# uncommitted6453/kzg-commitments

Hardware: AMD Instinct MI355X
Metric: KZG commits/sec + proofs/sec, BN254 degree-4096 (higher is better)
Workload: dtype u32 (radix-2^29 Montgomery limbs, 254-bit Fp)

## Files before the change

kzg-commitments_amd/csrc/coop.hpp:

```cpp
#pragma once
#include "curve.hpp"

namespace kzgx {

constexpr int COOP_G = 8;
constexpr int COOP_SLOTS = 40;

template <class F>
KZGX_DEV void f29_lds_st(uint32_t* p, const F29<F>& a) {
#pragma unroll
  for (int i = 0; i < F::L; i++) p[i] = a.v[i];
}
template <class F>
KZGX_DEV F29<F> f29_lds_ld(const uint32_t* p) {
  F29<F> a;
#pragma unroll
  for (int i = 0; i < F::L; i++) a.v[i] = p[i];
  return a;
}
KZGX_DEV void coop_fence() { __builtin_amdgcn_fence(__ATOMIC_SEQ_CST, "workgroup"); }

template <class F>
KZGX_DEV F29<F> f29_sel(bool c, const F29<F>& a, const F29<F>& b) {
  F29<F> r;
#pragma unroll
  for (int i = 0; i < F::L; i++) r.v[i] = c ? a.v[i] : b.v[i];
  return r;
}

template <class C>
KZGX_DEV Xyzz<C> coop_dbl(const Xyzz<C>& p, uint32_t* sc, int j) {
  using F = typename C::Fp29;
  constexpr int L = F::L;
  if (xyzz_is_inf<C>(p)) return p;
  uint32_t* b1 = sc;
  uint32_t* b2 = sc + 8 * L;
  uint32_t* b3 = sc + 16 * L;
  const F29<F> U = f29_add<F>(p.Y, p.Y);
  f29_lds_st<F>(b1 + j * L, f29_sqr<F>(f29_sel<F>(j == 0, U, p.X)));
  coop_fence();
  const F29<F> V = f29_lds_ld<F>(b1);
  const F29<F> xx = f29_lds_ld<F>(b1 + L);
  const F29<F> M = f29_add<F>(f29_add<F>(xx, xx), xx);
  {
    const F29<F> A = j == 0 ? U : j == 1 ? p.X : j == 2 ? M : V;
    const F29<F> B = j <= 1 ? V : j == 2 ? M : p.ZZ;
    f29_lds_st<F>(b2 + j * L, f29_mul<F>(A, B));
  }
  coop_fence();
  const F29<F> W = f29_lds_ld<F>(b2);
  const F29<F> S = f29_lds_ld<F>(b2 + L);
  const F29<F> X3 = f29_sub<F>(f29_lds_ld<F>(b2 + 2 * L), f29_add<F>(S, S), F::P4);
  {
    const F29<F> A = f29_sel<F>(j == 0, M, W);
    const F29<F> B = f29_sel<F>(j == 0, f29_sub<F>(S, X3, F::P8), p.ZZZ);
    const F29<F> Cc = f29_sel<F>(j == 0, W, f29_zero<F>());
    const F29<F> D = f29_sel<F>(j == 0, f29_sub<F>(f29_zero<F>(), p.Y, F::P4), f29_zero<F>());
    f29_lds_st<F>(b3 + j * L, f29_mul2<F>(A, B, Cc, D));
  }
  coop_fence();
  Xyzz<C> r;
  r.X = X3;
  r.Y = f29_lds_ld<F>(b3);
  r.ZZ = f29_lds_ld<F>(b2 + 3 * L);
  r.ZZZ = f29_lds_ld<F>(b3 + L);
  coop_fence();
  return r;
}

template <class C>
KZGX_DEV Xyzz<C> coop_add(const Xyzz<C>& p, const Xyzz<C>& q, uint32_t* sc, int j) {
  using F = typename C::Fp29;
  constexpr int L = F::L;
  if (xyzz_is_inf<C>(p)) return q;
  if (xyzz_is_inf<C>(q)) return p;
  uint32_t* b1 = sc;
  uint32_t* b2 = sc + 8 * L;
  uint32_t* b3 = sc + 16 * L;
  uint32_t* b4 = sc + 24 * L;
  uint32_t* bx = sc + 32 * L;
  {
    const F29<F> A = j == 0 ? p.X : j == 1 ? q.X : j == 2 ? p.Y : j == 3 ? q.Y : j == 4 ? p.ZZ : p.ZZZ;
    const F29<F> B = j == 0 ? q.ZZ : j == 1 ? p.ZZ : j == 2 ? q.ZZZ : j == 3 ? p.ZZZ : j == 4 ? q.ZZ : q.ZZZ;
    f29_lds_st<F>(b1 + j * L, f29_mul<F>(A, B));
  }
  coop_fence();
  {
    const int ia = (j & 1) ? 3 : 1;
    const F29<F> x = f29_sub<F>(f29_lds_ld<F>(b1 + ia * L), f29_lds_ld<F>(b1 + (ia - 1) * L), F::P2);
    f29_lds_st<F>(bx + j * L, x);
    f29_lds_st<F>(b2 + j * L, f29_sqr<F>(x));
  }
  coop_fence();
  const F29<F> PP = f29_lds_ld<F>(b2);
  if (f29_is_zero_lt2m<F>(PP)) {
    coop_fence();
    if (f29_is_zero<F>(f29_lds_ld<F>(bx + L))) return coop_dbl<C>(p, sc, j);
    return xyzz_inf<C>();
  }
  {
    const F29<F> A = j == 0 ? f29_lds_ld<F>(bx) : f29_lds_ld<F>(b1 + (j == 1 ? 0 : 4) * L);
    f29_lds_st<F>(b3 + j * L, f29_mul<F>(A, PP));
  }
  coop_fence();
  const F29<F> PPP = f29_lds_ld<F>(b3);
  const F29<F> Q = f29_lds_ld<F>(b3 + L);
  const F29<F> X3 = f29_sub<F>(f29_lds_ld<F>(b2 + L), f29_add<F>(PPP, f29_add<F>(Q, Q)), F::P6);
  {
    const F29<F> A = j == 0 ? f29_lds_ld<F>(bx + L) : f29_lds_ld<F>(b1 + 5 * L);
    const F29<F> B = f29_sel<F>(j == 0, f29_sub<F>(Q, X3, F::P8), PPP);
    const F29<F> Cc = f29_sel<F>(j == 0, f29_sub<F>(f29_zero<F>(), f29_lds_ld<F>(b1 + 2 * L), F::P2), f29_zero<F>());
    const F29<F> D = f29_sel<F>(j == 0, PPP, f29_zero<F>());
    f29_lds_st<F>(b4 + j * L, f29_mul2<F>(A, B, Cc, D));
  }
  coop_fence();
  Xyzz<C> r;
  r.X = X3;
  r.Y = f29_lds_ld<F>(b4);
  r.ZZ = f29_lds_ld<F>(b3 + 2 * L);
  r.ZZZ = f29_lds_ld<F>(b4 + L);
  coop_fence();
  return r;
}

}
```

kzg-commitments_amd/csrc/kzgx_api.hip:

```cpp
#include <hip/hip_runtime.h>

#include <map>
#include <mutex>

#include <array>

#include <algorithm>
#include <cstdlib>
#include <cstring>
#include <new>
#include <random>
#include <string>
#include <vector>

#include "curve_consts.h"
#include "fr_host.hpp"
#include "kzgx_internal.hpp"
#include "kzgx_setup.hpp"

#ifndef KZGX_G2TAB_EAGER_MAX
#define KZGX_G2TAB_EAGER_MAX 16385
#endif

struct kzgx_ctx {
// ... 346 lines not shown
  if (hipGetDeviceCount(&ndev) != hipSuccess || ndev <= 0) return KZGX_ERR_NO_DEVICE;
  if (device < 0 || device >= ndev) return KZGX_ERR_ARG;
  hipDeviceProp_t prop;
  KZGX_TRY_HIP(hipGetDeviceProperties(&prop, device));
  if (std::string(prop.gcnArchName).find("gfx950") == std::string::npos) return KZGX_ERR_NO_DEVICE;
  return KZGX_OK;
}

int setup_finish(kzgx_ctx* ctx);

}

extern "C" {

const char* kzgx_strerror(int s) {
  switch (s) {
    case KZGX_OK: return "ok";
    case KZGX_ERR_ARG: return "invalid argument";
    case KZGX_ERR_HIP: return "HIP runtime error";
    case KZGX_ERR_OOM: return "device out of memory";
    case KZGX_ERR_NO_SRS: return "no SRS loaded";
    case KZGX_ERR_DEGREE: return "polynomial degree be at most one less than the setup size (num_coeffs)";
    case KZGX_ERR_INTERNAL: return "internal error";
    case KZGX_ERR_NO_DEVICE: return "no gfx950 (MI355X) device available";
    case KZGX_ERR_DIV_ZERO: return "division by zero (duplicate interpolation point)";
    default: return "unknown status";
  }
}

int kzgx_base_limbs(int curve) {
  return curve == KZGX_CURVE_BN254 ? 4 : curve == KZGX_CURVE_BLS12381 ? 6 : -1;
}

namespace {
std::mutex g_stream_mu;
std::vector<hipStream_t> g_stream_pool[64];
constexpr size_t STREAM_POOL_MAX = 4;
hipError_t stream_take(int device, hipStream_t* s) {
  if (device >= 0 && device < 64) {
    std::lock_guard<std::mutex> lk(g_stream_mu);
    if (!g_stream_pool[device].empty()) {
      *s = g_stream_pool[device].back();
      g_stream_pool[device].pop_back();
      return hipSuccess;
    }
  }
  return hipStreamCreateWithFlags(s, hipStreamNonBlocking);
}
void stream_give(int device, hipStream_t s) {
  if (!s) return;
  if (device >= 0 && device < 64) {
    std::lock_guard<std::mutex> lk(g_stream_mu);
    if (g_stream_pool[device].size() < STREAM_POOL_MAX) {
      g_stream_pool[device].push_back(s);
      return;
    }
  }
  (void)hipStreamDestroy(s);
}
}

int kzgx_init_device(int curve, int device) {
  if (curve != KZGX_CURVE_BN254 && curve != KZGX_CURVE_BLS12381) return KZGX_ERR_ARG;
  KZGX_TRY(device_ok(device));
  KZGX_TRY_HIP(hipSetDevice(device));
  hipStream_t spare[3] = {nullptr, nullptr, nullptr};
  for (auto& s2 : spare) KZGX_TRY_HIP(stream_take(device, &s2));
  for (auto s2 : spare) stream_give(device, s2);
  hipStream_t st = nullptr;
  KZGX_TRY_HIP(stream_take(device, &st));
  struct StreamGuard {
    hipStream_t s;
    int d;
    ~StreamGuard() {
      (void)hipStreamSynchronize(s);
      stream_give(d, s);
    }
  } sg{st, device};
  int (*const warm[])(hipStream_t) = {
      kzgx::warm_setup,      kzgx::warm_msm,        kzgx::warm_msm_fixed,   kzgx::warm_poly,
      kzgx::warm_srs,        kzgx::warm_pairing,    kzgx::warm_verify_wave, kzgx::warm_latency,
      kzgx::warm_fixed_bn_a, kzgx::warm_fixed_bn_b, kzgx::warm_fixed_bn_c,  kzgx::warm_fixed_bn_d,
      kzgx::warm_fixed_bls_a, kzgx::warm_fixed_bls_b, kzgx::warm_fixed_bls_c, kzgx::warm_fixed_bls_d,
      kzgx::warm_subgroup,   kzgx::warm_msm_joint};
  for (auto f : warm) KZGX_TRY(f(st));
  kzgx::GenTables g;
  KZGX_TRY(kzgx::gen_tables_get(curve, device, st, &g));
  void* h = nullptr;
  KZGX_TRY_HIP(hipHostMalloc(&h, 4096, hipHostMallocMapped | hipHostMallocCoherent));
  (void)hipHostFree(h);
  KZGX_TRY_HIP(hipStreamSynchronize(st));
  return KZGX_OK;
}

int kzgx_create(kzgx_ctx** out, int curve, int device) {
  if (!out || (curve != KZGX_CURVE_BN254 && curve != KZGX_CURVE_BLS12381)) return KZGX_ERR_ARG;
  *out = nullptr;
  KZGX_TRY(device_ok(device));
  kzgx_ctx* ctx = new (std::nothrow) kzgx_ctx();
  if (!ctx) return KZGX_ERR_OOM;
  ctx->c.curve = curve;
  ctx->c.device = device;
  if (const char* e = getenv("KZGX_WINDOW_BITS")) {
    int c = atoi(e);
    if (kzgx::window_bits_supported(c)) ctx->c.c = c;
  }
  ctx->c.W = (257 + ctx->c.c - 1) / ctx->c.c;
  ctx->c.fixed.joint.g_req = -1;
  if (const char* e = getenv("KZGX_FIXED_JOINT")) {
    const int g = atoi(e);
    if (g == -1 || g == 0 || (g >= 2 && g <= 25)) ctx->c.fixed.joint.g_req = g;
  }
  if (const char* e = getenv("KZGX_FIXED_JOINT_RANGES")) {
    const int r = atoi(e);
    if (r >= 0 && r <= 8) ctx->c.fixed.joint.ranges = (uint32_t)r;
  }
  hipError_t e = hipSetDevice(device);
  if (e == hipSuccess) e = stream_take(device, &ctx->c.stream);
  if (e != hipSuccess) {
    delete ctx;
    return kzgx::hip_fail(e);
  }
  kzgx::ctx_live_add(device, +1);
  *out = ctx;
  return KZGX_OK;
}

int kzgx_release_cached_memory(int device) {
  if (device < 0 || device >= 64) return KZGX_ERR_ARG;
  int prev = 0;
  KZGX_TRY_HIP(hipGetDevice(&prev));
  KZGX_TRY_HIP(hipSetDevice(device));
  kzgx::table_cache_release();
  return hipSetDevice(prev) == hipSuccess ? KZGX_OK : KZGX_ERR_HIP;
}

int kzgx_shared_tables(int device, size_t* count, size_t* bytes) {
  if (!count || !bytes || device < 0 || device >= 64) return KZGX_ERR_ARG;
  kzgx::shared_tables_info(device, count, bytes);
  return KZGX_OK;
}

void kzgx_destroy(kzgx_ctx* ctx) {
  if (!ctx) return;
  (void)hipSetDevice(ctx->c.device);
  (void)hipStreamSynchronize(ctx->c.stream);
  (void)kzgx_prof_clear(ctx);
  Ctx& c = ctx->c;
  void* bufs[] = {c.d_table, c.d_table_small, c.d_table_big, c.d_inf, c.d_stage[0], c.d_stage[1], c.d_stage[2], c.d_stage[3],
                  c.d_poly_ws, c.d_poly_ws2, ctx->d_srs_canon, ctx->d_srs2_canon, c.d_g2_ws, ctx->d_vw, ctx->d_g2tab,
                  c.d_lift, c.d_ntt_tw};
  for (void* p : bufs)
    if (p) (void)hipFree(p);
  for (void* p : ctx->d_chk)
    if (p) (void)hipFree(p);
  for (auto& f : c.fk) {
    if (f.x) (void)hipFree(f.x);
    if (f.inf) (void)hipFree(f.inf);
    if (f.ev) (void)hipEventDestroy(f.ev);
  }
  for (auto& row : c.fkm)
    for (auto& f : row) {
      if (f.x) (void)hipFree(f.x);
      if (f.inf) (void)hipFree(f.inf);
      if (f.ev) (void)hipEventDestroy(f.ev);
    }
  kzgx::fixed_free(&c);
// ... 2087 lines not shown
```

kzg-commitments_amd/csrc/kzgx_internal.hpp:

```cpp
#pragma once
#include <hip/hip_runtime.h>
#include <stddef.h>
#include <stdint.h>

#include <cstdlib>
#include <vector>

#include "../../include/kzg_gpu.h"

#ifndef KZGX_ACCUM_WAVES
#define KZGX_ACCUM_WAVES 3
#endif

#ifndef KZGX_BS_WAVES
#define KZGX_BS_WAVES 2
#endif

#ifndef KZGX_WINDOW_BITS
#define KZGX_WINDOW_BITS 12
#endif

#define KZGX_TRY(expr)                 \
  do {                                 \
    int _rc = (expr);                  \
// ... 185 lines not shown
      if (w.bound_at < lru->bound_at) lru = &w;
    if (lru->done_recorded && hipEventSynchronize(lru->done) != hipSuccess) return WsLease(this, nullptr, st);
    lru->done_recorded = false;
    lru->owner = st;
    lru->bound_at = ++ws_clock;
    return WsLease(this, lru, st);
  }
  void ws_release(MsmWs* w, hipStream_t st) {
    if (!w->done && hipEventCreateWithFlags(&w->done, hipEventDisableTiming) != hipSuccess) {
      w->done = nullptr;
      (void)hipStreamSynchronize(st);
      return;
    }
    w->done_recorded = hipEventRecord(w->done, st) == hipSuccess;
    if (!w->done_recorded) (void)hipStreamSynchronize(st);
  }
  bool prof_on = false;
  std::vector<ProfRec> prof;
  void* d_poly_ws = nullptr;
  size_t poly_ws_b = 0;
  void* d_poly_ws2 = nullptr;
  size_t poly_ws2_b = 0;
  void* d_g2_ws = nullptr;
  size_t g2_ws_b = 0;
  uint32_t* d_lift = nullptr;
  size_t lift_b = 0;
  uint32_t* d_ntt_tw = nullptr;
  size_t ntt_tw_b = 0;
  int ntt_log2 = -1;
  hipEvent_t ntt_ev = nullptr;
  FkSetup fk[NTT_MAX_LOG2];
  FkSetup fkm[NTT_MAX_LOG2 + 1][NTT_MAX_LOG2 + 1];
  void* d_stage[4] = {nullptr, nullptr, nullptr, nullptr};
  size_t stage_b[4] = {0, 0, 0, 0};
  int base_words() const { return curve == KZGX_CURVE_BN254 ? 8 : 12; }
};

inline WsLease::~WsLease() {
  if (w_) c_->ws_release(w_, st_);
}

struct ProfScope {
  Ctx* ctx;
  hipStream_t st;
  ProfRec rec;
  ProfScope(Ctx* c, hipStream_t s, const char* name) : ctx(c), st(s) {
    rec.name = nullptr;
    if (!ctx->prof_on) return;
    rec.name = name;
    (void)hipEventCreate(&rec.a);
    (void)hipEventCreate(&rec.b);
    (void)hipEventRecord(rec.a, st);
  }
  ~ProfScope() {
    if (!rec.name) return;
    (void)hipEventRecord(rec.b, st);
    ctx->prof.push_back(rec);
  }
};

int dev_alloc(Ctx* ctx, void** p, size_t bytes, size_t* cap);

bool window_bits_supported(int c);
bool fixed_bits_supported(int c);
int fixed_windows(int curve, int c);
int fixed_build(Ctx* ctx, const uint32_t* d_canon, size_t n_srs);
int fixed_build_table(Ctx* ctx, FixedTable& ft, const uint32_t* d_canon, size_t n_srs);
int fixed_rebuild_default(Ctx* ctx, const uint32_t* d_canon, size_t n_srs);
void fixed_free(Ctx* ctx);
void fixed_free_table(FixedTable& ft);
bool fixed_usable(const Ctx* ctx, size_t n);
bool fixed_table_usable(const FixedTable& ft, size_t n);
int fixed_msm_table(Ctx* ctx, FixedTable& ft, const uint32_t* d_scalars, size_t n, size_t batch, size_t stride_words,
                    uint32_t* d_out, uint32_t* d_out_inf, hipStream_t st, uint32_t* xyzz_out);
int fixed_msm(Ctx* ctx, const uint32_t* d_scalars, size_t n, size_t batch, size_t stride_words, uint32_t* d_out,
              uint32_t* d_out_inf, hipStream_t st, uint32_t* xyzz_out);
size_t joint_table_bytes(int curve, int g, size_t n);
int joint_plan(int curve, int c, size_t n, int g_req, int* g, int* c_win);
int joint_build(Ctx* ctx, JointTable& jt, const uint32_t* d_canon, size_t n, int g);
void joint_free(JointTable& jt);
bool joint_serves(const FixedTable& ft, size_t n, size_t batch, bool xyzz_out);
int joint_msm(Ctx* ctx, FixedTable& ft, const uint32_t* d_scalars, size_t n, size_t batch, size_t stride_words,
              uint32_t* d_out, uint32_t* d_out_inf, hipStream_t st);
int srs_upload(Ctx* ctx, const uint32_t* d_canon, size_t n);
int microbench_mixed_add(Ctx* ctx, double* rate);
int microbench_mad_u64(Ctx* ctx, double* rate, double* ghz);
int clock_probe(Ctx* ctx, hipStream_t st, uint32_t spin_us, uint64_t* d_out);
size_t fixed_table_bytes(int curve, int c, size_t n);
int debug_latency(Ctx* ctx, int op, uint32_t iters, double* res);
int xyzz_sum(Ctx* ctx, const uint32_t* d_parts, size_t count, uint32_t* d_out, uint32_t* d_out_inf, hipStream_t st);
int msm_batch(Ctx* ctx, const uint32_t* d_scalars, size_t n, size_t batch, size_t stride_words, uint32_t* d_out,
              uint32_t* d_out_inf, hipStream_t st);
struct PointSeg {
  const uint32_t* xy;
  const uint32_t* inf;
  size_t n;
};
constexpr size_t MSM_POINTS_MAX = KZGX_MSM_POINTS_MAX;
int msm_points(Ctx* ctx, MsmWs& ws, const PointSeg* segs, int nseg, const uint32_t* d_scalars, uint32_t* d_out,
               uint32_t* d_out_inf, hipStream_t st);
int aggregate_scalars(Ctx* ctx, const uint32_t* d_z, const uint32_t* d_y, const uint32_t* d_r, size_t n,
                      uint32_t* d_out, hipStream_t st);
size_t cells_fold_slices(size_t count, unsigned log2l);
int cells_scalars(Ctx* ctx, const uint32_t* d_T, const uint32_t* d_r, const uint32_t* d_cell_index,
                  const uint32_t* d_commit_index, size_t count, size_t n_commits, unsigned log2l, unsigned log2D,
                  bool bitrev, uint32_t* d_out, uint32_t* d_gate, hipStream_t st);
int msm_partial_xyzz(Ctx* ctx, const uint32_t* d_scalars, size_t n, uint32_t* d_rec, hipStream_t st);
int gen_srs_points(Ctx* ctx, const uint32_t* tau_canon_host, size_t start, size_t n, uint32_t* d_out_canon,
                   hipStream_t st);
int g1_validate(Ctx* ctx, const uint32_t* d_xy, uint32_t* d_ok, hipStream_t st);
int g1_sum(Ctx* ctx, const uint32_t* d_xy, const uint32_t* d_inf, size_t count, uint32_t* d_out, uint32_t* d_out_inf,
           hipStream_t st);

int quotient_single(Ctx* ctx, const uint32_t* d_coeffs, size_t n, size_t coeff_stride_words, const uint32_t* d_z,
                    size_t batch, uint32_t* d_q, size_t q_stride_words, uint32_t* d_y, hipStream_t st);
int poly_eval(Ctx* ctx, const uint32_t* d_coeffs, size_t n, const uint32_t* d_x, size_t m, uint32_t* d_y,
              hipStream_t st);
int poly_vanishing(Ctx* ctx, const uint32_t* d_x, size_t n, uint32_t* d_Z, hipStream_t st);
int prove_range_poly(Ctx* ctx, const uint32_t* d_P, size_t n, const uint32_t* d_x, size_t len, uint32_t* d_q,
                     size_t* nq, hipStream_t st);
int poly_interpolate(Ctx* ctx, const uint32_t* d_x, const uint32_t* d_y, size_t n, uint32_t* d_coeffs,
                     hipStream_t st);
int verify_ws_reserve(Ctx* ctx, size_t n);
int g2_ws_reserve(Ctx* ctx, size_t n);

int ntt_max_log2(int curve);
int ntt(Ctx* ctx, const uint32_t* d_in, size_t in_stride, uint32_t* d_out, size_t out_stride, unsigned log2n,
        size_t batch, bool inverse, bool bitrev, hipStream_t st);
int ntt_twiddles(Ctx* ctx, unsigned log2n, hipStream_t st);

int g1_ntt(Ctx* ctx, MsmWs& ws, const uint32_t* d_in_xy, const uint32_t* d_in_inf, uint32_t* d_out_xy,
           uint32_t* d_out_inf, unsigned log2n, size_t batch, bool inverse, bool bitrev, hipStream_t st);
int prove_all_setup(Ctx* ctx, MsmWs& ws, const uint32_t* d_srs_canon, unsigned log2n, hipStream_t st);
int prove_all(Ctx* ctx, MsmWs& ws, const uint32_t* d_srs_canon, const uint32_t* d_coeffs, size_t stride,
              unsigned log2n, size_t batch, bool bitrev, uint32_t* d_out_xy, uint32_t* d_out_inf, hipStream_t st);
void prove_all_drop(Ctx* ctx);
int prove_cosets_setup(Ctx* ctx, MsmWs& ws, const uint32_t* d_srs_canon, unsigned log2n, unsigned log2l,
                       hipStream_t st);
int prove_cosets(Ctx* ctx, MsmWs& ws, const uint32_t* d_srs_canon, const uint32_t* d_coeffs, size_t stride,
                 unsigned log2n, unsigned log2l, size_t batch, bool ext, bool bitrev, uint32_t* d_out_xy,
                 uint32_t* d_out_inf, uint32_t* d_y, hipStream_t st);

constexpr size_t RECOVER_CHUNK_SCALARS = KZGX_RECOVER_CHUNK_SCALARS;
int recover_cells(Ctx* ctx, MsmWs& ws, const uint32_t* d_blob_index, const uint32_t* d_cell_index,
                  const uint32_t* d_ys, size_t count, size_t n_blobs, size_t b0, size_t cb, unsigned log2n,
                  unsigned log2l, bool bitrev, bool want_coef, uint32_t* d_out_y, uint32_t* d_out_coeffs,
                  uint32_t* d_ok, hipStream_t st);

int gen_srs_g2_points(Ctx* ctx, const uint32_t* d_tau, size_t start, size_t n, uint32_t* d_out, hipStream_t st);
size_t g2_table_bytes(int curve, size_t n);
int g2_table_build(Ctx* ctx, const uint32_t* d_srs2, size_t n, uint32_t* d_tab, hipStream_t st);
int msm_g2(Ctx* ctx, const uint32_t* d_scalars, const uint32_t* d_srs2, size_t n, uint32_t* d_out,
           uint32_t* d_out_inf, hipStream_t st,
           const uint32_t* d_tab = nullptr);
int g2_validate(Ctx* ctx, const uint32_t* d_xy, size_t count, uint32_t* d_ok, hipStream_t st);
int pairing_batch(Ctx* ctx, const uint32_t* d_g1, const uint32_t* d_g1_inf, const uint32_t* d_g2,
                  const uint32_t* d_g2_inf, size_t count, uint32_t* d_out, hipStream_t st);
int verify_single_batch(Ctx* ctx, const uint32_t* d_commits, const uint32_t* d_commit_inf, const uint32_t* d_proofs,
                        const uint32_t* d_proof_inf, const uint32_t* d_z, const uint32_t* d_y, size_t count,
                        const uint32_t* d_g1_0, const uint32_t* d_g2_01, uint32_t* d_ok, hipStream_t st);
size_t verify_wave_bytes(int curve);
int verify_wave_prepare(Ctx* ctx, const uint32_t* d_g1_0, const uint32_t* d_g2_01, const uint32_t* g1_comb,
                        uint32_t* d_buf, hipStream_t st);
int verify_wave_batch(Ctx* ctx, const uint32_t* d_commits, const uint32_t* d_commit_inf, const uint32_t* d_proofs,
                      const uint32_t* d_proof_inf, const uint32_t* d_z, const uint32_t* d_y, size_t count,
                      const uint32_t* d_g1_0, const uint32_t* d_buf, uint32_t* d_ok, hipStream_t st);
// ... 18 lines not shown
```

kzg-commitments_amd/csrc/kzgx_setup.hpp:

```cpp
#pragma once
#include <hip/hip_runtime.h>

#include <cstddef>
#include <cstdint>

namespace kzgx {

int warm_setup(hipStream_t st);
int warm_msm(hipStream_t st);
int warm_msm_fixed(hipStream_t st);
int warm_poly(hipStream_t st);
int warm_srs(hipStream_t st);
int warm_pairing(hipStream_t st);
int warm_verify_wave(hipStream_t st);
int warm_latency(hipStream_t st);
int warm_subgroup(hipStream_t st);
int warm_msm_joint(hipStream_t st);
int warm_fixed_bn_a(hipStream_t st);
int warm_fixed_bn_b(hipStream_t st);
int warm_fixed_bn_c(hipStream_t st);
int warm_fixed_bn_d(hipStream_t st);
int warm_fixed_bls_a(hipStream_t st);
int warm_fixed_bls_b(hipStream_t st);
int warm_fixed_bls_c(hipStream_t st);
int warm_fixed_bls_d(hipStream_t st);

struct GenTables {
  uint32_t* g1_comb = nullptr;
  uint32_t* g2_comb = nullptr;
};
constexpr int GEN_COMB_ENTRIES = 32 * 255;
int gen_tables_get(int curve, int device, hipStream_t st, GenTables* out);

int gen_srs_g1_comb(int curve, const uint32_t* d_tau, size_t start, size_t n, const uint32_t* g1_comb,
                    uint32_t* d_out, hipStream_t st);
int gen_srs_g2_comb(int curve, const uint32_t* d_tau, size_t start, size_t n, const uint32_t* g2_comb,
                    uint32_t* d_out, hipStream_t st);

int fixed_multiples_batch(int curve, const uint32_t* d_bases, const uint8_t* d_inf, uint32_t n, int W, uint32_t H,
                          size_t is, size_t ws, uint32_t* d_tab, hipStream_t st);

int vtab_prepare(int curve, const uint32_t* d_g1_0, const uint32_t* g1_comb, uint32_t* d_vtab, hipStream_t st);

int g1_fold_packed(int curve, const uint32_t* d_rec, size_t count, uint32_t* d_out, hipStream_t st);
#ifndef KZGX_G2_TAB_BITS
#define KZGX_G2_TAB_BITS 8
#endif
constexpr int G2_TAB_BITS = KZGX_G2_TAB_BITS;
static_assert(G2_TAB_BITS == 4 || G2_TAB_BITS == 8 || G2_TAB_BITS == 16, "digits must tile a 32-bit word");
constexpr int G2_TAB_WINDOWS = 256 / G2_TAB_BITS;
int g2_table_comb(int curve, const uint32_t* d_tau, size_t start, size_t n, const uint32_t* g2_comb, uint32_t* d_tab,
                  hipStream_t st);
size_t xyzz_record_words(int curve);
int g1_fold_xyzz(int curve, const uint32_t* d_rec, size_t count, uint32_t* d_out, hipStream_t st);
int affine_to_xyzz(int curve, const uint32_t* d_xy, const uint32_t* d_inf, uint32_t* d_rec, hipStream_t st);

int vw_bench(int curve, int op, uint32_t iters, double* ns_per_op, double* clk_per_op, hipStream_t st);

size_t big_reduce_rt_bytes(int curve, uint32_t nb);
int big_reduce(int curve, const uint32_t* d_offsets, uint32_t nb, const uint32_t* d_bsum, uint32_t* d_rt,
               uint32_t* d_out, uint32_t* d_out_inf, hipStream_t st, uint32_t* xyzz_out = nullptr);
int big_reduce_seg(int curve, const uint32_t* d_seg_off, uint32_t* d_part, uint32_t nb, uint32_t s_ub,
                   const uint32_t* d_flag, uint32_t* d_rt, uint32_t* d_out, uint32_t* d_out_inf, hipStream_t st,
                   uint32_t* xyzz_out = nullptr);

}
```

kzg-commitments_amd/csrc/msm_joint.hip:

```cpp
#include <hip/hip_runtime.h>

#include <algorithm>

#include "curve.hpp"
#include "fixed_accum.hpp"
#include "fixed_msm.hpp"
#include "kzgx_internal.hpp"
#include "kzgx_setup.hpp"

namespace kzgx {

constexpr uint32_t JOINT_PL = 256;
constexpr uint32_t JOINT_NEG = 1u << 31;

__host__ __device__ static inline int joint_split(int m) { return m < 4 ? m : (m / 2 > 4 ? m / 2 : 4); }

template <class F>
KZGX_DEV void f29_store_words(uint32_t* p, const F29<F>& a) {
#pragma unroll
  for (int i = 0; i < F::L; i++) p[i] = a.v[i];
}
template <class F>
KZGX_DEV F29<F> f29_load_words(const uint32_t* p) {
  F29<F> r;
#pragma unroll
  for (int i = 0; i < F::L; i++) r.v[i] = p[i];
  return r;
}

size_t joint_table_bytes(int curve, int g, size_t n) {
  if (g < 2 || n == 0) return 0;
  const size_t pb = curve == KZGX_CURVE_BN254 ? packed_words<BN254G1>() * 4 : packed_words<BLS12381G1>() * 4;
  return (n + g - 1) / g * ((size_t)1 << (g - 1)) * pb;
}

template <class C>
__global__ __launch_bounds__(64) void k_joint_halves(const uint32_t* __restrict__ canon, uint32_t n_t, uint32_t g,
                                                     uint32_t blocks, uint32_t la_max, uint32_t hs,
                                                     uint32_t* __restrict__ half) {
  constexpr int AW = affine_words<C>();
  const uint64_t t = (uint64_t)blockIdx.x * blockDim.x + threadIdx.x;
  if (t >= (uint64_t)blocks * hs) return;
  const uint32_t b = (uint32_t)(t / hs), e = (uint32_t)(t % hs);
  const uint32_t p0 = b * g;
  const uint32_t gb = n_t - p0 < g ? n_t - p0 : g;
  const int m = (int)gb - 1, a = joint_split(m);
  const bool hi = e >= la_max;
  const uint32_t j = hi ? e - la_max : e;
  const int cnt = hi ? m - a : a;
  if (j >= (1u << cnt)) return;
  Xyzz<C> acc = xyzz_inf<C>();
  Affine<C> p;
  if (hi && affine_from_canonical<C>(canon + (size_t)(p0 + m) * 2 * C::Fp::N, p)) acc = xyzz_from_affine<C>(p);
  const uint32_t first = p0 + (hi ? (uint32_t)a : 0u);
  for (int i = 0; i < cnt; i++) {
    if (!affine_from_canonical<C>(canon + (size_t)(first + i) * 2 * C::Fp::N, p)) continue;
    if (!((j >> i) & 1u)) p = affine_neg<C>(p);
    acc = xyzz_add_affine<C>(acc, p);
  }
  xyzz_to_affine<C>(acc, p);
  affine_store<C>(half + ((size_t)b * hs + e) * AW, p);
}

template <class C>
KZGX_DEV bool affine_is_inf(const Affine<C>& a) {
  using F = typename C::Fp29;
  return f29_is_zero_exact<F>(a.x) && f29_is_zero_exact<F>(a.y);
}

template <class C>
KZGX_PT bool joint_entry_exact(const Affine<C>& hb, const Affine<C>& la, Affine<C>& out) {
  Xyzz<C> s = affine_is_inf<C>(hb) ? xyzz_inf<C>() : xyzz_from_affine<C>(hb);
  if (!affine_is_inf<C>(la)) s = xyzz_add_affine<C>(s, la);
  return xyzz_to_affine<C>(s, out);
}

template <class C>
__global__ __launch_bounds__(64) void k_joint_entries_small(const uint32_t* __restrict__ half, uint32_t b0,
                                                            uint32_t nb, int m, uint32_t la_max, uint32_t hs,
                                                            size_t bstride, uint32_t* __restrict__ tab,
                                                            unsigned long long* __restrict__ n_inf) {
  constexpr int AW = affine_words<C>();
  constexpr int PW = packed_words<C>();
  const int a = joint_split(m);
  const uint64_t t = (uint64_t)blockIdx.x * blockDim.x + threadIdx.x;
  if (t >= ((uint64_t)nb << m)) return;
  const uint32_t b = b0 + (uint32_t)(t >> m), j = (uint32_t)(t & ((1u << m) - 1u));
  const uint32_t* H = half + (size_t)b * hs * AW;
  Affine<C> r;
  const bool fin = joint_entry_exact<C>(affine_load<C>(H + (size_t)(la_max + (j >> a)) * AW),
                                        affine_load<C>(H + (size_t)(j & ((1u << a) - 1u)) * AW), r);
  if (!fin) atomicAdd(n_inf, 1ull);
  packed_store<C>(tab + (size_t)b * bstride + (size_t)j * PW, r);
}

// ... 178 lines not shown
  constexpr int BITS = C::SCALAR_BITS;
  const uint32_t b = blockIdx.y, lane = threadIdx.x;
  const uint32_t hi = lane >> 5, li = lane & 31u;
  const uint32_t blk = 2 * blockIdx.x + hi;
  uint32_t gb = 0;
  if (blk < nb) gb = n_t - blk * g < g ? n_t - blk * g : g;
  const uint32_t i = blk * g + li;
  uint32_t s[8] = {0, 0, 0, 0, 0, 0, 0, 0};
  if (li < gb && i < n) scalar_load(scalars + (size_t)b * stride_words + (size_t)i * 8, s);
  scalar_reduce<C>(s);
  const uint32_t flip = odd_prepare<C>(s);
  s[(BITS - 1) >> 5] |= 1u << ((BITS - 1) & 31);
  const uint32_t keep = li < gb ? ~0u : 0u;
#pragma unroll
  for (int k = 0; k < 8; k++) s[k] = (s[k] ^ (0u - flip)) & keep;
  const uint32_t low = gb ? (1u << (gb - 1)) - 1u : 0u;
  uint32_t* out = idx + ((size_t)b * nb + blk) * JOINT_PL + li;
#pragma unroll
  for (int k = 0; k < 8; k++) {
    uint32_t mine = s[k];
    auto swap = [&](int j, uint32_t m) __attribute__((always_inline)) {
      const uint32_t p = __shfl_xor(mine, j, 64);
      mine = (li & (uint32_t)j) ? (((p >> j) & m) | (mine & ~m)) : ((mine & m) | ((p & m) << j));
    };
    swap(16, 0x0000ffffu);
    swap(8, 0x00ff00ffu);
    swap(4, 0x0f0f0f0fu);
    swap(2, 0x33333333u);
    swap(1, 0x55555555u);
    if (gb) {
      const uint32_t top = (mine >> (gb - 1)) & 1u;
      out[32 * k] = ((top ? mine : ~mine) & low) | (top ? 0u : JOINT_NEG);
    }
  }
}

template <class C, bool INF, int V = madd_variant<C>()>
__global__ __launch_bounds__(64, fixed_accum_waves<C>()) void k_joint_accum(
    const uint32_t* __restrict__ idx, uint32_t nb, uint32_t per, const uint32_t* __restrict__ tab, size_t bstride,
    uint32_t R, uint32_t* __restrict__ part) {
  constexpr int XW = xyzz_words<C>();
  constexpr int PW = packed_words<C>();
  const uint32_t b = blockIdx.y, rho = blockIdx.x >> 2;
  const uint32_t w = (blockIdx.x & 3u) * 64 + threadIdx.x;
  if (w >= (uint32_t)C::SCALAR_BITS) return;
  const uint32_t b0 = rho * per, b1 = b0 + per < nb ? b0 + per : nb;
  Xyzz<C> acc = xyzz_inf<C>();
  if (b0 < b1) {
    const uint32_t last = b1 - 1;
    const uint32_t* ip = idx + (size_t)b * nb * JOINT_PL + w;
    auto fetch = [&](uint32_t blk, uint32_t word) __attribute__((always_inline)) {
      return packed_fetch<C>(tab + (size_t)blk * bstride + (size_t)(word & ~JOINT_NEG) * PW);
    };
    uint32_t wq = ip[(size_t)b0 * JOINT_PL];
    PackedPt<C> pq = fetch(b0, wq);
    uint32_t wn = ip[(size_t)(b0 + 1 < last ? b0 + 1 : last) * JOINT_PL];
#pragma unroll 1
    for (uint32_t blk = b0; blk < b1; blk++) {
      Affine<C> cur = packed_unpack<C>(pq);
      const uint32_t neg = wq >> 31;
      const uint32_t nx = blk + 1 < last ? blk + 1 : last;
      wq = wn;
      pq = fetch(nx, wq);
      wn = ip[(size_t)(blk + 2 < last ? blk + 2 : last) * JOINT_PL];
      const bool skip = INF && affine_is_inf<C>(cur);
      affine_cond_neg<C>(cur, neg);
      const Xyzz<C> sum = xyzz_add_affine_v<C, V>(acc, cur);
      if constexpr (INF) {
#pragma unroll
        for (int k = 0; k < C::Fp29::L; k++) {
          acc.X.v[k] = skip ? acc.X.v[k] : sum.X.v[k];
          acc.Y.v[k] = skip ? acc.Y.v[k] : sum.Y.v[k];
          acc.ZZ.v[k] = skip ? acc.ZZ.v[k] : sum.ZZ.v[k];
          acc.ZZZ.v[k] = skip ? acc.ZZZ.v[k] : sum.ZZZ.v[k];
        }
      } else {
        acc = sum;
      }
    }
  }
  xyzz_store<C>(part + (((size_t)b * R + rho) * JOINT_PL + w) * XW, acc);
}

template <class C>
__global__ __launch_bounds__(64) void k_joint_horner1(const uint32_t* __restrict__ part, uint32_t count,
                                                      uint32_t* __restrict__ segs) {
  constexpr int XW = xyzz_words<C>();
  constexpr uint32_t BITS = C::SCALAR_BITS;
  const uint32_t t = blockIdx.x * blockDim.x + threadIdx.x;
  if (t >= count * 8) return;
  const uint32_t br = t >> 3, seg = t & 7u;
  const uint32_t lo = 32 * seg, hi = lo + 32 < BITS ? lo + 32 : BITS;
  const uint32_t* p = part + (size_t)br * JOINT_PL * XW;
  Xyzz<C> acc = xyzz_load<C>(p + (size_t)(hi - 1) * XW);
  for (uint32_t w = hi - 1; w-- > lo;) {
    const Xyzz<C> a = xyzz_load<C>(p + (size_t)w * XW);
    acc = xyzz_dbl<C>(acc);
    acc = xyzz_add<C>(acc, a);
  }
  xyzz_store<C>(segs + (size_t)t * XW, acc);
}

template <class C>
__global__ __launch_bounds__(64) void k_joint_horner2(const uint32_t* __restrict__ segs, uint32_t batch, uint32_t R,
                                                      uint32_t* __restrict__ sums) {
  constexpr int XW = xyzz_words<C>();
  const uint32_t b = blockIdx.x * blockDim.x + threadIdx.x;
  if (b >= batch) return;
  const uint32_t* p = segs + (size_t)b * R * 8 * XW;
  Xyzz<C> acc = xyzz_inf<C>();
  for (int seg = 7; seg >= 0; seg--) {
    if (seg < 7)
      for (int k = 0; k < 32; k++) acc = xyzz_dbl<C>(acc);
    for (uint32_t r = 0; r < R; r++) acc = xyzz_add<C>(acc, xyzz_load<C>(p + ((size_t)r * 8 + seg) * XW));
  }
  xyzz_store<C>(sums + (size_t)b * XW, acc);
}

bool joint_serves(const FixedTable& ft, size_t n, size_t batch, bool xyzz_out) {
  const JointTable& jt = ft.joint;
  if (!jt.d || xyzz_out || n == 0 || n > jt.n_t) return false;
  return jt.g_req >= 2 ? batch >= 1 : batch >= 64;
}

template <class C>
static int joint_msm_impl(Ctx* ctx, FixedTable& ft, const uint32_t* d_scalars, size_t n, size_t batch,
                          size_t stride_words, uint32_t* d_out, uint32_t* d_out_inf, hipStream_t st) {
  const JointTable& jt = ft.joint;
  constexpr size_t XB = xyzz_words<C>() * sizeof(uint32_t);
  static_assert(C::SCALAR_BITS <= (int)JOINT_PL && C::SCALAR_BITS > 224, "4 wavefronts and 8 segments of planes");
  const uint32_t nb = (uint32_t)((n + jt.g - 1) / jt.g);
  uint32_t R = jt.ranges ? jt.ranges : 1u;
  R = std::min(R, nb);
  const uint32_t per = (nb + R - 1) / R;
  if (batch > 65535 || 4 * (size_t)R > 65535) return KZGX_ERR_ARG;
  WsLease wsp = ctx->ws_for(st);
  if (!wsp) return KZGX_ERR_ARG;
  MsmWs& ws = *wsp;
  KZGX_TRY(dev_alloc(ctx, (void**)&ws.jidx, batch * (size_t)nb * JOINT_PL * 4, &ws.jidx_b));
  KZGX_TRY(dev_alloc(ctx, (void**)&ws.fpart, batch * (size_t)R * JOINT_PL * XB, &ws.fpart_b));
  KZGX_TRY(dev_alloc(ctx, (void**)&ws.fsum, batch * ((size_t)R * 8 + 1) * XB, &ws.fsum_b));
  {
    ProfScope p(ctx, st, "msm_scatter");
    hipLaunchKernelGGL(k_joint_index<C>, dim3((nb + 1) / 2, (unsigned)batch), dim3(64), 0, st, d_scalars, (uint32_t)n,
                       stride_words, (uint32_t)jt.n_t, (uint32_t)jt.g, nb, ws.jidx);
  }
  {
    ProfScope p(ctx, st, "msm_accum");
    const size_t bstride = ((size_t)1 << (jt.g - 1)) * packed_words<C>();
    if (jt.n_inf)
      hipLaunchKernelGGL((k_joint_accum<C, true>), dim3(4 * R, (unsigned)batch), dim3(64), 0, st, ws.jidx, nb, per,
                         jt.d, bstride, R, ws.fpart);
    else
      hipLaunchKernelGGL((k_joint_accum<C, false>), dim3(4 * R, (unsigned)batch), dim3(64), 0, st, ws.jidx, nb, per,
                         jt.d, bstride, R, ws.fpart);
  }
  {
    ProfScope p(ctx, st, "msm_reduce");
    uint32_t* sums = ws.fsum + batch * (size_t)R * 8 * xyzz_words<C>();
    hipLaunchKernelGGL(k_joint_horner1<C>, dim3((unsigned)((batch * R * 8 + 63) / 64)), dim3(64), 0, st, ws.fpart,
                       (uint32_t)(batch * R), ws.fsum);
    hipLaunchKernelGGL(k_joint_horner2<C>, dim3((unsigned)((batch + 63) / 64)), dim3(64), 0, st, ws.fsum,
                       (uint32_t)batch, R, sums);
    fixed_finish_launch<C>(sums, (uint32_t)batch, d_out, d_out_inf, nullptr, st);
  }
  KZGX_TRY_HIP(hipGetLastError());
  return KZGX_OK;
}

int joint_msm(Ctx* ctx, FixedTable& ft, const uint32_t* d_scalars, size_t n, size_t batch, size_t stride_words,
              uint32_t* d_out, uint32_t* d_out_inf, hipStream_t st) {
  return ctx->curve == KZGX_CURVE_BN254
             ? joint_msm_impl<BN254G1>(ctx, ft, d_scalars, n, batch, stride_words, d_out, d_out_inf, st)
             : joint_msm_impl<BLS12381G1>(ctx, ft, d_scalars, n, batch, stride_words, d_out, d_out_inf, st);
}

__global__ void k_warm_msm_joint() {}
int warm_msm_joint(hipStream_t st) {
  hipLaunchKernelGGL(k_warm_msm_joint, dim3(1), dim3(64), 0, st);
  KZGX_TRY_HIP(hipGetLastError());
  return KZGX_OK;
}

}
```

Before: 284,800.

## Split joint Horner into 16 segments and cooperative 8-lane final reduce

The joint MSM's Horner reduction now splits the 256 bit-planes into 16 segments of 16 instead of 8 of 32, doubling parallelism in the first pass. The second pass, previously one thread per batch item running serial doublings and adds, now uses groups of 8 lanes that cooperate on each point doubling and addition through LDS. This shortens the serial tail that leaves the GPU underused at small batch. The cost is more segment partials to combine, LDS fences on every group operation, and a separate compile unit that needs special memory-clause flags.

```diff
diff --git a/kzg-commitments_amd/csrc/coop.hpp b/kzg-commitments_amd/csrc/coop.hpp
--- a/kzg-commitments_amd/csrc/coop.hpp
+++ b/kzg-commitments_amd/csrc/coop.hpp
@@ -43,8 +43,8 @@
   const F29<F> xx = f29_lds_ld<F>(b1 + L);
   const F29<F> M = f29_add<F>(f29_add<F>(xx, xx), xx);
   {
-    const F29<F> A = j == 0 ? U : j == 1 ? p.X : j == 2 ? M : V;
-    const F29<F> B = j <= 1 ? V : j == 2 ? M : p.ZZ;
+    const F29<F> A = f29_sel<F>(j == 0, U, f29_sel<F>(j == 1, p.X, f29_sel<F>(j == 2, M, V)));
+    const F29<F> B = f29_sel<F>(j <= 1, V, f29_sel<F>(j == 2, M, p.ZZ));
     f29_lds_st<F>(b2 + j * L, f29_mul<F>(A, B));
   }
   coop_fence();
@@ -80,8 +80,12 @@
   uint32_t* b4 = sc + 24 * L;
   uint32_t* bx = sc + 32 * L;
   {
-    const F29<F> A = j == 0 ? p.X : j == 1 ? q.X : j == 2 ? p.Y : j == 3 ? q.Y : j == 4 ? p.ZZ : p.ZZZ;
-    const F29<F> B = j == 0 ? q.ZZ : j == 1 ? p.ZZ : j == 2 ? q.ZZZ : j == 3 ? p.ZZZ : j == 4 ? q.ZZ : q.ZZZ;
+    const F29<F> A = f29_sel<F>(
+        j == 0, p.X,
+        f29_sel<F>(j == 1, q.X, f29_sel<F>(j == 2, p.Y, f29_sel<F>(j == 3, q.Y, f29_sel<F>(j == 4, p.ZZ, p.ZZZ)))));
+    const F29<F> B = f29_sel<F>(
+        j == 0, q.ZZ,
+        f29_sel<F>(j == 1, p.ZZ, f29_sel<F>(j == 2, q.ZZZ, f29_sel<F>(j == 3, p.ZZZ, f29_sel<F>(j == 4, q.ZZ, q.ZZZ)))));
     f29_lds_st<F>(b1 + j * L, f29_mul<F>(A, B));
   }
   coop_fence();
diff --git a/kzg-commitments_amd/csrc/joint_horner.hip b/kzg-commitments_amd/csrc/joint_horner.hip
--- /dev/null
+++ b/kzg-commitments_amd/csrc/joint_horner.hip
@@ -0,0 +1,85 @@
+#ifndef KZGX_MEMCLAUSE_OFF
+#error "joint_horner.hip needs -mllvm -amdgpu-max-memory-clause=1 -DKZGX_MEMCLAUSE_OFF (see the Makefile)"
+#endif
+#include <hip/hip_runtime.h>
+
+#include "coop.hpp"
+#include "curve.hpp"
+#include "kzgx_internal.hpp"
+#include "kzgx_setup.hpp"
+
+namespace kzgx {
+
+template <class C>
+__global__ __launch_bounds__(64) void k_joint_horner1(const uint32_t* __restrict__ part, uint64_t lanes,
+                                                      uint32_t* __restrict__ segs) {
+  constexpr int XW = xyzz_words<C>();
+  constexpr uint32_t BITS = C::SCALAR_BITS;
+  const uint64_t t = (uint64_t)blockIdx.x * blockDim.x + threadIdx.x;
+  if (t >= lanes) return;
+  const uint64_t br = t / JOINT_NSEG;
+  const uint32_t seg = (uint32_t)(t % JOINT_NSEG);
+  const uint32_t lo = JOINT_SEG * seg, hi = lo + JOINT_SEG < BITS ? lo + JOINT_SEG : BITS;
+  const uint32_t* p = part + br * JOINT_PL * XW;
+  Xyzz<C> acc = xyzz_load<C>(p + (size_t)(hi - 1) * XW);
+  for (uint32_t w = hi - 1; w-- > lo;) {
+    const Xyzz<C> a = xyzz_load<C>(p + (size_t)w * XW);
+    acc = xyzz_dbl<C>(acc);
+    acc = xyzz_add<C>(acc, a);
+  }
+  xyzz_store<C>(segs + t * XW, acc);
+}
+
+template <class C>
+__global__ __launch_bounds__(64) void k_joint_horner2(const uint32_t* __restrict__ segs, uint32_t batch, uint32_t R,
+                                                      uint32_t* __restrict__ sums) {
+  constexpr int XW = xyzz_words<C>();
+  constexpr int L = C::Fp29::L;
+  __shared__ uint32_t sc[(64 / COOP_G) * COOP_SLOTS * L];
+  const uint32_t grp = threadIdx.x / COOP_G;
+  const int j = (int)(threadIdx.x % COOP_G);
+  const uint32_t b = blockIdx.x * (64 / COOP_G) + grp;
+  if (b >= batch) return;
+  uint32_t* my = sc + grp * COOP_SLOTS * L;
+  const uint32_t* p = segs + (size_t)b * R * JOINT_NSEG * XW;
+  auto seg_sum = [&](uint32_t r, uint32_t seg) __attribute__((always_inline)) {
+    return xyzz_load<C>(p + ((size_t)r * JOINT_NSEG + seg) * XW);
+  };
+  Xyzz<C> acc = seg_sum(0, JOINT_NSEG - 1);
+#pragma unroll 1
+  for (uint32_t r = 1; r < R; r++) acc = coop_add<C>(acc, seg_sum(r, JOINT_NSEG - 1), my, j);
+#pragma unroll 1
+  for (uint32_t seg = JOINT_NSEG - 1; seg-- > 0;) {
+    const Xyzz<C> nxt = seg_sum(0, seg);
+#pragma unroll 1
+    for (uint32_t k = 0; k < JOINT_SEG; k++) acc = coop_dbl<C>(acc, my, j);
+    acc = coop_add<C>(acc, nxt, my, j);
+#pragma unroll 1
+    for (uint32_t r = 1; r < R; r++) acc = coop_add<C>(acc, seg_sum(r, seg), my, j);
+  }
+  if (j == 0) xyzz_store<C>(sums + (size_t)b * XW, acc);
+}
+
+template <class C>
+int joint_horner_launch(const uint32_t* part, uint32_t batch, uint32_t R, uint32_t* segs, uint32_t* sums,
+                        hipStream_t st) {
+  static_assert(C::SCALAR_BITS <= (int)JOINT_PL && C::SCALAR_BITS > (int)(JOINT_PL - JOINT_SEG),
+                "the top segment holds at least one plane");
+  const uint64_t lanes = (uint64_t)batch * R * JOINT_NSEG;
+  if (batch == 0 || R == 0 || (lanes + 63) / 64 > 0x7fffffffull) return KZGX_ERR_ARG;
+  hipLaunchKernelGGL(k_joint_horner1<C>, dim3((unsigned)((lanes + 63) / 64)), dim3(64), 0, st, part, lanes, segs);
+  constexpr uint32_t GPW = 64 / COOP_G;
+  hipLaunchKernelGGL(k_joint_horner2<C>, dim3((batch + GPW - 1) / GPW), dim3(64), 0, st, segs, batch, R, sums);
+  return KZGX_OK;
+}
+template int joint_horner_launch<BN254G1>(const uint32_t*, uint32_t, uint32_t, uint32_t*, uint32_t*, hipStream_t);
+template int joint_horner_launch<BLS12381G1>(const uint32_t*, uint32_t, uint32_t, uint32_t*, uint32_t*, hipStream_t);
+
+__global__ void k_warm_joint_horner() {}
+int warm_joint_horner(hipStream_t st) {
+  hipLaunchKernelGGL(k_warm_joint_horner, dim3(1), dim3(64), 0, st);
+  KZGX_TRY_HIP(hipGetLastError());
+  return KZGX_OK;
+}
+
+}
diff --git a/kzg-commitments_amd/csrc/kzgx_api.hip b/kzg-commitments_amd/csrc/kzgx_api.hip
--- a/kzg-commitments_amd/csrc/kzgx_api.hip
+++ b/kzg-commitments_amd/csrc/kzgx_api.hip
@@ -452,7 +452,7 @@
       kzgx::warm_srs,        kzgx::warm_pairing,    kzgx::warm_verify_wave, kzgx::warm_latency,
       kzgx::warm_fixed_bn_a, kzgx::warm_fixed_bn_b, kzgx::warm_fixed_bn_c,  kzgx::warm_fixed_bn_d,
       kzgx::warm_fixed_bls_a, kzgx::warm_fixed_bls_b, kzgx::warm_fixed_bls_c, kzgx::warm_fixed_bls_d,
-      kzgx::warm_subgroup,   kzgx::warm_msm_joint};
+      kzgx::warm_subgroup,   kzgx::warm_msm_joint,  kzgx::warm_joint_horner};
   for (auto f : warm) KZGX_TRY(f(st));
   kzgx::GenTables g;
   KZGX_TRY(kzgx::gen_tables_get(curve, device, st, &g));
diff --git a/kzg-commitments_amd/csrc/kzgx_internal.hpp b/kzg-commitments_amd/csrc/kzgx_internal.hpp
--- a/kzg-commitments_amd/csrc/kzgx_internal.hpp
+++ b/kzg-commitments_amd/csrc/kzgx_internal.hpp
@@ -291,6 +291,13 @@
 bool joint_serves(const FixedTable& ft, size_t n, size_t batch, bool xyzz_out);
 int joint_msm(Ctx* ctx, FixedTable& ft, const uint32_t* d_scalars, size_t n, size_t batch, size_t stride_words,
               uint32_t* d_out, uint32_t* d_out_inf, hipStream_t st);
+constexpr uint32_t JOINT_PL = 256;
+constexpr uint32_t JOINT_SEG = 16;
+constexpr uint32_t JOINT_NSEG = JOINT_PL / JOINT_SEG;
+static_assert(JOINT_NSEG * JOINT_SEG == JOINT_PL, "whole segments");
+template <class C>
+int joint_horner_launch(const uint32_t* part, uint32_t batch, uint32_t R, uint32_t* segs, uint32_t* sums,
+                        hipStream_t st);
 int srs_upload(Ctx* ctx, const uint32_t* d_canon, size_t n);
 int microbench_mixed_add(Ctx* ctx, double* rate);
 int microbench_mad_u64(Ctx* ctx, double* rate, double* ghz);
diff --git a/kzg-commitments_amd/csrc/kzgx_setup.hpp b/kzg-commitments_amd/csrc/kzgx_setup.hpp
--- a/kzg-commitments_amd/csrc/kzgx_setup.hpp
+++ b/kzg-commitments_amd/csrc/kzgx_setup.hpp
@@ -16,6 +16,7 @@
 int warm_latency(hipStream_t st);
 int warm_subgroup(hipStream_t st);
 int warm_msm_joint(hipStream_t st);
+int warm_joint_horner(hipStream_t st);
 int warm_fixed_bn_a(hipStream_t st);
 int warm_fixed_bn_b(hipStream_t st);
 int warm_fixed_bn_c(hipStream_t st);
diff --git a/kzg-commitments_amd/csrc/msm_joint.hip b/kzg-commitments_amd/csrc/msm_joint.hip
--- a/kzg-commitments_amd/csrc/msm_joint.hip
+++ b/kzg-commitments_amd/csrc/msm_joint.hip
@@ -10,7 +10,6 @@
 
 namespace kzgx {
 
-constexpr uint32_t JOINT_PL = 256;
 constexpr uint32_t JOINT_NEG = 1u << 31;
 
 __host__ __device__ static inline int joint_split(int m) { return m < 4 ? m : (m / 2 > 4 ? m / 2 : 4); }
@@ -355,40 +354,6 @@
   xyzz_store<C>(part + (((size_t)b * R + rho) * JOINT_PL + w) * XW, acc);
 }
 
-template <class C>
-__global__ __launch_bounds__(64) void k_joint_horner1(const uint32_t* __restrict__ part, uint32_t count,
-                                                      uint32_t* __restrict__ segs) {
-  constexpr int XW = xyzz_words<C>();
-  constexpr uint32_t BITS = C::SCALAR_BITS;
-  const uint32_t t = blockIdx.x * blockDim.x + threadIdx.x;
-  if (t >= count * 8) return;
-  const uint32_t br = t >> 3, seg = t & 7u;
-  const uint32_t lo = 32 * seg, hi = lo + 32 < BITS ? lo + 32 : BITS;
-  const uint32_t* p = part + (size_t)br * JOINT_PL * XW;
-  Xyzz<C> acc = xyzz_load<C>(p + (size_t)(hi - 1) * XW);
-  for (uint32_t w = hi - 1; w-- > lo;) {
-    const Xyzz<C> a = xyzz_load<C>(p + (size_t)w * XW);
-    acc = xyzz_dbl<C>(acc);
-    acc = xyzz_add<C>(acc, a);
-  }
-  xyzz_store<C>(segs + (size_t)t * XW, acc);
-}
-
-template <class C>
-__global__ __launch_bounds__(64) void k_joint_horner2(const uint32_t* __restrict__ segs, uint32_t batch, uint32_t R,
-                                                      uint32_t* __restrict__ sums) {
-  constexpr int XW = xyzz_words<C>();
-  const uint32_t b = blockIdx.x * blockDim.x + threadIdx.x;
-  if (b >= batch) return;
-  const uint32_t* p = segs + (size_t)b * R * 8 * XW;
-  Xyzz<C> acc = xyzz_inf<C>();
-  for (int seg = 7; seg >= 0; seg--) {
-    if (seg < 7)
-      for (int k = 0; k < 32; k++) acc = xyzz_dbl<C>(acc);
-    for (uint32_t r = 0; r < R; r++) acc = xyzz_add<C>(acc, xyzz_load<C>(p + ((size_t)r * 8 + seg) * XW));
-  }
-  xyzz_store<C>(sums + (size_t)b * XW, acc);
-}
 
 bool joint_serves(const FixedTable& ft, size_t n, size_t batch, bool xyzz_out) {
   const JointTable& jt = ft.joint;
@@ -401,7 +366,7 @@
                           size_t stride_words, uint32_t* d_out, uint32_t* d_out_inf, hipStream_t st) {
   const JointTable& jt = ft.joint;
   constexpr size_t XB = xyzz_words<C>() * sizeof(uint32_t);
-  static_assert(C::SCALAR_BITS <= (int)JOINT_PL && C::SCALAR_BITS > 224, "4 wavefronts and 8 segments of planes");
+  static_assert(C::SCALAR_BITS <= (int)JOINT_PL && C::SCALAR_BITS > 192, "4 wavefronts of planes");
   const uint32_t nb = (uint32_t)((n + jt.g - 1) / jt.g);
   uint32_t R = jt.ranges ? jt.ranges : 1u;
   R = std::min(R, nb);
@@ -412,7 +377,7 @@
   MsmWs& ws = *wsp;
   KZGX_TRY(dev_alloc(ctx, (void**)&ws.jidx, batch * (size_t)nb * JOINT_PL * 4, &ws.jidx_b));
   KZGX_TRY(dev_alloc(ctx, (void**)&ws.fpart, batch * (size_t)R * JOINT_PL * XB, &ws.fpart_b));
-  KZGX_TRY(dev_alloc(ctx, (void**)&ws.fsum, batch * ((size_t)R * 8 + 1) * XB, &ws.fsum_b));
+  KZGX_TRY(dev_alloc(ctx, (void**)&ws.fsum, batch * ((size_t)R * JOINT_NSEG + 1) * XB, &ws.fsum_b));
   {
     ProfScope p(ctx, st, "msm_scatter");
     hipLaunchKernelGGL(k_joint_index<C>, dim3((nb + 1) / 2, (unsigned)batch), dim3(64), 0, st, d_scalars, (uint32_t)n,
@@ -430,11 +395,8 @@
   }
   {
     ProfScope p(ctx, st, "msm_reduce");
-    uint32_t* sums = ws.fsum + batch * (size_t)R * 8 * xyzz_words<C>();
-    hipLaunchKernelGGL(k_joint_horner1<C>, dim3((unsigned)((batch * R * 8 + 63) / 64)), dim3(64), 0, st, ws.fpart,
-                       (uint32_t)(batch * R), ws.fsum);
-    hipLaunchKernelGGL(k_joint_horner2<C>, dim3((unsigned)((batch + 63) / 64)), dim3(64), 0, st, ws.fsum,
-                       (uint32_t)batch, R, sums);
+    uint32_t* sums = ws.fsum + batch * (size_t)R * JOINT_NSEG * xyzz_words<C>();
+    KZGX_TRY(joint_horner_launch<C>(ws.fpart, (uint32_t)batch, R, ws.fsum, sums, st));
     fixed_finish_launch<C>(sums, (uint32_t)batch, d_out, d_out_inf, nullptr, st);
   }
   KZGX_TRY_HIP(hipGetLastError());
```

After: 304,900, median of 6. 1.07x the previous value.
